# 3b/3bz

Hardware: AMD Instinct MI355X
Metric: decompressed MB/s on 1 GiB many-block zlib, 1/2/4/8 MI355X; % HBM roofline (higher is better)
Workload: dtype u8

## Files before the change

3bz_amd/csrc/tbz_engine.hpp:

```cpp
#pragma once
#include <algorithm>
#include <atomic>
#include <chrono>
#include <condition_variable>
#include <mutex>
#include <cstdio>
#include <cstdlib>
#include <cstring>
#include <functional>
#include <memory>
#include <string>
#include <thread>
#include <utility>
#include <vector>

#include "../../include/tbz_amd.h"
#include "tbz_kernels.hpp"

static_assert(sizeof(tbz_result) == 64, "tbz_result is exchanged between ranks as 64-octet records");
namespace tbz {

struct DevBuf {
  void* p = nullptr;
  size_t cap = 0;
};

}

#define TBZ_CTX_POOLS(X) \
  X(d_str_off) X(d_str_len) X(d_tile_first) X(d_tile_counts) X(d_tile_offsets) X(d_markers) X(d_items) X(d_res) \
  X(d_tok) X(d_scratch) X(d_runs) X(d_segs) X(d_groups) X(d_order) X(d_k3_fi) X(d_k3_ni) \
  X(d_k3_oo) X(d_k3_oc) X(d_k3_sums) X(d_k3_flags) X(d_k3_gscan) X(d_k3_gne) X(d_k3_streams) X(d_k3_glob) \
  X(d_redo_items) X(d_redo_res) X(d_k0_slots) X(d_k0_fm) X(d_hdr) X(d_gck) X(d_gchunks) X(d_ck_l1) \
  X(d_tok2) X(d_runs2) X(d_ck_chunks) X(d_ck_parts) X(d_ck_streams) X(d_ck_out) X(d_crc_tab) X(d_in_stage) \
  X(d_out_stage) X(d_kb_tf) X(d_kb_slots) X(d_kb_counts) X(d_kb_offsets) X(d_kb_cands) X(d_kb_fc) X(d_kb_head) \
  X(d_markers2) X(d_kb_fm2) X(d_mark) X(d_hg) X(d_k6s) X(d_bigs) X(d_recs) X(d_kc_tf) \
  X(d_kc_slots) X(d_kc_ends) X(d_kc_link) X(d_kc_fm2) X(d_markers3) X(d_kb_keep) X(d_kb_kcounts) X(d_gz_cands) \
  X(d_gz_count) X(d_gz_tmp) X(d_wide_res) X(d_cold) X(d_cold2) X(d_small_rec) \
  X(d_bit_off) X(d_ix_span) X(d_ix_recs) X(d_rec_pieces) X(d_rec_queries) X(d_rec_out) \
  X(d_srch_pieces) X(d_srch_flags) X(d_srch_hits)

namespace tbz {
static inline void cpu_relax() {
#if defined(__x86_64__) || defined(__i386__)
  __builtin_ia32_pause();
#else
  std::this_thread::yield();
// ... 72 lines not shown
      std::lock_guard<std::mutex> lk(mu);
      stop = true;
    }
    cv.notify_all();
    for (auto& t : th) t.join();
  }
};
}

struct tbz_ctx {
  int device = 0;
  hipStream_t stream = nullptr;
  hipStream_t stream2 = nullptr;
  hipEvent_t evw[2] = {};
  hipEvent_t ev[12] = {};
  std::string err;
  tbz_timings tim{};
  uint64_t gang_rounds = 0, gang_valid = 0;
  bool k1h = true;
  bool k2_ring2 = false;
  bool k2_single = false;
  bool host_layout = false;
  void* h_pin = nullptr;
  size_t h_pin_cap = 0;
  void* h_stage[4] = {};
  hipEvent_t ev_stage[4] = {};
  tbz::CopyPool* copy_pool = nullptr;
  tbz::CopyPool* copy_pool2 = nullptr;
  hipStream_t stream_in = nullptr, stream_out = nullptr;
  bool small_fused = true;
// ... 424 lines not shown
    R->trailer_isize = format == TBZ_FORMAT_GZIP ? q.trailer1 : 0u;
    (format == TBZ_FORMAT_ZLIB ? R->adler32 : R->crc32) = h->check;
  }
  ctx->tim.huff_launches = 1;
  ctx->tim.k1_gang = 64;
  ctx->tim.k2_kinds = q.tok_words ? 4u : 0u;
  ctx->tim.token_words = q.tok_words;
  ctx->tim.n_segments = ctx->tim.n_groups = R->segments;
  ctx->tim.scratch_bytes = scratch_total(ctx);
  ctx->gang_rounds = q.reserved >> 32;
  ctx->gang_valid = q.reserved & 0xffffffffu;
  *handled = true;
  return 0;
}

static void launch_k2_linear(tbz_ctx* ctx, K2Params& k2, size_t n_groups, uint64_t max_out) {
  k2.win_bytes = (u32)((max_out + K2_SLACK + 63) & ~63ull);
  ctx->tim.k2_kinds |= ctx->k2_single ? 2u : 1u;
  if (ctx->k2_single)
    TBZ_LAUNCH_DYN(tbz_k2_lz77_small, n_groups, k2.win_bytes + 2 * K2_TOKBUF + 512, ctx->stream, k2);
  else
    TBZ_LAUNCH_DYN_WG(tbz_k2_lz77_dual, n_groups, 128, k2.win_bytes + 2 * K2_TOKBUF + 512 + 2 * sizeof(K2Hand),
                      ctx->stream, k2);
}
static void launch_k2_ring(tbz_ctx* ctx, const K2Params& k2, size_t nwg) {
  ctx->tim.k2_kinds |= 4u;
  if (ctx->k2_single) TBZ_LAUNCH(tbz_k2_lz77, nwg, ctx->stream, k2);
  else if (ctx->k2_ring2) TBZ_LAUNCH_WG(tbz_k2_lz77_ring2, nwg, 128, ctx->stream, k2);
  else TBZ_LAUNCH_WG(tbz_k2_lz77_ring3, nwg, 192, ctx->stream, k2);
}
static void k2_trace(tbz_ctx* ctx) {
#ifdef TBZ_WAVE_TRACE
  if (const char* vp = getenv("TBZ_K2_TRACE")) {
    std::vector<u64> h(8192 * 8);
    hipStreamSynchronize(ctx->stream);
    u32 cn[4] = {0, 0, 0, 0};
    hipMemcpyFromSymbol(cn, HIP_SYMBOL(tbz_dbg_cnt), 16);
    fprintf(stderr, "tbz: K2 resolve since the start: %u batches with matches, %.2f rounds and %.1f matches per batch\n", cn[0],
            cn[0] ? (double)cn[1] / cn[0] : 0.0, cn[0] ? (double)cn[2] / cn[0] : 0.0);
    hipMemcpyFromSymbol(h.data(), HIP_SYMBOL(tbz_dbg), h.size() * 8);
    if (FILE* f = fopen(vp, "wb")) { fwrite(h.data(), 8, h.size(), f); fclose(f); }
  }
#endif
}
// ... 119 lines not shown
    if (total / count >= (uint64_t)ctx->tun.k6_lds_min) {
      q.pieces = (u32)((maxlen + 15 + K6R_PIECE - 1) / K6R_PIECE);
      TBZ_LAUNCH_WG(tbz_k6_resolve_lds, count * (size_t)q.pieces, K6R_THREADS, ctx->stream, q);
    } else {
      q.pieces = (u32)((maxlen + 15 + K6_PIECE - 1) / K6_PIECE);
      TBZ_LAUNCH(tbz_k6_resolve, count * (size_t)q.pieces, ctx->stream, q);
    }
  };
  resolve(o3s, r3s, K6_W);
  resolve(o3a, r3a, K6_W);
  resolve(o3b, r3b, 65536);
  TBZ_HIP(hipEventRecord(ctx->ev[11], ctx->stream));
  return 0;
}

enum { DIST_NONE = 0, DIST_FIRST = 1, DIST_AFTER_OVERFLOW = 2 };
struct Call {
  tbz_ctx* ctx;
  int format;
  size_t n;
  const void* d_in;
  const uint64_t *in_offs, *in_lens;
  void* d_out;
  const uint64_t *out_offs, *out_caps;
  tbz_result* results;
  bool size_only;
  CoreOpts* opt;
  std::vector<uint64_t> hist;
  std::vector<uint32_t> bit_off;
  const u32* d_bit_off = nullptr;
// ... 5 lines not shown
  std::vector<StreamPlan> sp;
  uint64_t tiles = 0, in_lo = ~0ull, in_extent = 0, in_total_bits = 0;
  uint32_t n_mark = 0, n_fixed_items = 0;
  uint32_t n_stored_heads = 0;
  std::vector<uint32_t> first_marker;
  const u64* d_markers_cur = nullptr;
  const u32* d_first_marker = nullptr;
  size_t n_items = 0;
  std::vector<Item> items;
  bool have_find = false;
  uint64_t pool_base = 0, pool2_base = 0, pool2_hi = 0;
  u32 half1 = 0, half2 = 0;
  bool wide_beside = false;
  float huff_ms = 0;
  bool simple = false;
  K3Params k3{};
  K3Global* h_glob = nullptr;
  K3Stream* h_k3s = nullptr;
  bool fused_adler = false;
  std::vector<std::vector<SegHost>> per_stream;
  std::vector<uint8_t> dist_first;
  uint64_t dist_at = ~0ull;
  std::vector<Seg> h_segs;
  std::vector<Group> h_groups;
  std::vector<uint8_t> h_hist;
  std::vector<uint32_t> h_gstream;
  std::vector<int32_t> h_grec;
  std::vector<BigSeg> bigs;
  uint32_t n_recs = 0;
};
// ... 66 lines not shown
    S.in_len = c.in_lens[s];
    S.out_off = c.size_only ? 0 : c.out_offs[s];
    S.out_cap = c.size_only ? ~0ull : c.out_caps[s];
    c.in_extent = std::max(c.in_extent, c.in_offs[s] + c.in_lens[s]);
    if (c.in_lens[s]) c.in_lo = std::min(c.in_lo, c.in_offs[s]);
    c.in_total_bits += c.in_lens[s] * 8;
    tile_first[s] = (uint32_t)c.tiles;
    c.tiles += ((((uintptr_t)c.d_in + c.in_offs[s]) & 15) + c.in_lens[s] + SCAN_TILE - 1) / SCAN_TILE;
    if (c.tiles > 0x7fffffffu) return TBZ_E_ARG;
  }
  tile_first[n] = (uint32_t)c.tiles;
  if (c.in_extent && !c.d_in) return TBZ_E_ARG;
  const size_t tiles = c.tiles;
  int r;
  if ((r = record(ctx, 0))) return r;
  if ((r = pinned(ctx, (n + 5) * 4 + 16 + sizeof(K3Global) + (n + 1) * sizeof(K3Stream)))) return r;
  if (tiles) {
    const std::vector<uint64_t> h_off(c.in_offs, c.in_offs + n), h_len(c.in_lens, c.in_lens + n);
    if ((r = upload(ctx, ctx->d_str_off, h_off))) return r;
    if ((r = upload(ctx, ctx->d_str_len, h_len))) return r;
    if ((r = upload(ctx, ctx->d_tile_first, tile_first))) return r;
    if ((r = ensure(ctx, ctx->d_tile_counts, tiles * 4))) return r;
    if ((r = ensure(ctx, ctx->d_tile_offsets, (tiles + 1) * 4))) return r;
    if ((r = ensure(ctx, ctx->d_k0_slots, tiles * (size_t)K0_SLOTS * 8))) return r;
    if ((r = ensure(ctx, ctx->d_markers, tiles * (size_t)K0_SLOTS * 8 + 16))) return r;
    if ((r = ensure(ctx, ctx->d_k0_fm, (n + 1) * 4 + 16))) return r;
    if ((r = ensure(ctx, ctx->d_items, (tiles * (size_t)K0_SLOTS + n) * sizeof(Item)))) return r;
    if (!c.bit_off.empty()) {
      if ((r = upload(ctx, ctx->d_bit_off, c.bit_off))) return r;
      c.d_bit_off = (const u32*)ctx->d_bit_off.p;
    }
// ... 241 lines not shown
  }
  return 0;
}
static u32 items_per_wg(size_t n_it) {
  u32 ipw = 64;
  while (ipw > 1 && n_it / ipw < 512) ipw >>= 1;
  return ipw;
}
static u32 pool_half(const Call& c, bool fix) { return fix ? c.half2 : c.half1; }
static u16* pool_tok(const Call& c, bool fix) {
  return fix ? (u16*)c.ctx->d_tok2.p - ((c.pool2_base >> c.half2) & ~7ull) : (u16*)c.ctx->d_tok.p - ((c.pool_base >> c.half1) & ~7ull);
}
static RunRec* pool_runs(const Call& c, bool fix) {
  return fix ? (RunRec*)c.ctx->d_runs2.p - (c.pool2_base >> RUN_SHIFT) : (RunRec*)c.ctx->d_runs.p - (c.pool_base >> RUN_SHIFT);
}
static int launch_lane(Call& c, const Item* d_items, SegResult* d_res, size_t n_it, bool fix, bool explicit_items = false) {
  tbz_ctx* ctx = c.ctx;
  if (pool_half(c, fix) && !explicit_items) return TBZ_E_INTERNAL;
  int rr = ensure(ctx, ctx->d_scratch, n_it * (size_t)K1_SCRATCH);
  if (rr) return rr;
  K1Params k1{(const u8*)c.d_in, pool_tok(c, fix), d_items, d_res, c.d_markers_cur,
              (u8*)ctx->d_scratch.p, pool_runs(c, fix), c.d_first_marker, (u32)c.n_mark, (u32)n_it, items_per_wg(n_it), c.resume_abs};
  TBZ_LAUNCH(tbz_k1_huff_decode, (n_it + k1.items_per_wg - 1) / k1.items_per_wg, ctx->stream, k1);
  return 0;
}
static u32 sub_min(const tbz_ctx* ctx) {
  if (ctx->tun.sub_min) return (u32)std::max(64, ctx->tun.sub_min & ~63);
  return KG_SUB_MIN;
}
static u64 wide_for(const tbz_ctx* ctx, int G, bool fix) {
  if (ctx->tun.wide_bits >= 0) return (u64)ctx->tun.wide_bits;
  if (ctx->k1_mode || fix || G >= 64) return 0;
  return (u64)G * KG_SUB_MAX * 2;
}
static u32 ovl_for(const tbz_ctx* ctx, int G) {
  if (ctx->tun.ovl) return (u32)std::max(64, ctx->tun.ovl);
  return G >= 32 ? 1024u : 768u;
}
// ... 38 lines not shown
    if (sub.empty()) continue;
    if (ctx->tun.debug && how == REDO_GANG) {
      uint64_t mx = 0;
      for (const Item& q : sub) mx = std::max<uint64_t>(mx, std::min(q.limit_bit, q.end_byte * 8) - q.start_bit);
      fprintf(stderr, "tbz: %zu large item(s) handed to gangs of 64 (the largest: %llu bits)\n", sub.size(), (unsigned long long)mx);
    }
    if (ctx->tun.debug && how == REDO_GANG_OWN) fprintf(stderr, "tbz: %zu item(s) decoded again into regions of their own\n", sub.size());
    if (ctx->tun.debug && how == REDO_LANE) fprintf(stderr, "tbz: %zu item(s) redone by the one-lane kernel\n", sub.size());
    std::vector<SegResult> tmp;
    int r;
    if ((r = k1_again(c, sub, how, fix, tmp))) return r;
    for (size_t k = 0; k < idx.size(); k++) rs[idx[k]] = tmp[k];
  }
  return 0;
}
static int launch_k1(Call& c, const Item* d_items, SegResult* d_res, size_t n_it, bool fix) {
  tbz_ctx* ctx = c.ctx;
  int G = k1_gang(c, n_it);
  if (G == 1 && pool_half(c, fix)) G = 8;
  if (!fix) ctx->tim.k1_gang = (uint32_t)G;
  if (G == 1) return launch_lane(c, d_items, d_res, n_it, fix);
  size_t per = 64 / G, nwg = (n_it + per - 1) / per;
  if (!fix && G <= 16 && wide_for(ctx, G, fix) && ctx->stream2) {
    int rr = ensure(ctx, ctx->d_wide_res, n_it * sizeof(SegResult));
    if (rr) return rr;
    if ((rr = ensure(ctx, ctx->d_cold2, n_it * (size_t)KG_COLD_STRIDE))) return rr;
    TBZ_HIP(hipEventRecord(ctx->evw[0], ctx->stream));
    TBZ_HIP(hipStreamWaitEvent(ctx->stream2, ctx->evw[0], 0));
    K1gParams kw = k1g_params(c, d_items, (SegResult*)ctx->d_wide_res.p, n_it, 64, fix, false, (u8*)ctx->d_cold2.p);
    kw.only_wide = 1;
    kw.wide_bits = wide_for(ctx, G, fix);
    TBZ_LAUNCH(tbz_k1g64_huff_decode, n_it, ctx->stream2, kw);
    TBZ_HIP(hipEventRecord(ctx->evw[1], ctx->stream2));
    c.wide_beside = true;
  }
  int rr;
  if ((rr = ensure(ctx, ctx->d_scratch, n_it * (size_t)K1_SCRATCH))) return rr;
  if ((rr = ensure(ctx, ctx->d_hdr, n_it * sizeof(HdrRec)))) return rr;
  if (G >= 32 && (rr = ensure(ctx, ctx->d_cold, n_it * (size_t)KG_COLD_STRIDE))) return rr;
  K1hParams kh{(const u8*)c.d_in, d_items, (u8*)ctx->d_scratch.p, (HdrRec*)ctx->d_hdr.p, (u32)n_it};
  if (ctx->k1h) TBZ_LAUNCH(tbz_k1h_headers, (n_it + 63) / 64, ctx->stream, kh);
  K1gParams kg = k1g_params(c, d_items, d_res, n_it, G, fix, false, (u8*)ctx->d_cold.p);
  kg.hdr = ctx->k1h ? (const HdrRec*)ctx->d_hdr.p : nullptr;
  kg.hdr_lens = (const u8*)ctx->d_scratch.p;
  kg.wide_bits = wide_for(ctx, G, fix);
#ifdef TBZ_WAVE_TRACE
  {
    static int n_launch = 0;
    u32 ef = (n_launch++ >= 1 && getenv("TBZ_EXP")) ? (u32)atoi(getenv("TBZ_EXP")) : 0u;
    hipMemcpyToSymbolAsync(HIP_SYMBOL(tbz_exp_flags), &ef, 4, 0, hipMemcpyHostToDevice, ctx->stream);
    hipStreamSynchronize(ctx->stream);
  }
  static u64* d_trace = nullptr;
  static size_t trace_wg = 0;
  if (const char* tp = getenv("TBZ_WAVE_TRACE")) {
    if (d_trace && trace_wg) {
      std::vector<u64> h(trace_wg * 16);
      hipStreamSynchronize(ctx->stream);
      hipMemcpy(h.data(), d_trace, h.size() * 8, hipMemcpyDeviceToHost);
      if (FILE* f = fopen(tp, "wb")) { fwrite(h.data(), 8, h.size(), f); fclose(f); }
      hipFree(d_trace);
    }
    hipMalloc((void**)&d_trace, nwg * 128);
    hipMemsetAsync(d_trace, 0, nwg * 128, ctx->stream);
    trace_wg = nwg;
    kg.trace = d_trace;
  }
#endif
  switch (G) {
    case 8: TBZ_LAUNCH(tbz_k1g8_huff_decode, nwg, ctx->stream, kg); break;
    case 16: TBZ_LAUNCH(tbz_k1g16_huff_decode, nwg, ctx->stream, kg); break;
    case 32: TBZ_LAUNCH(tbz_k1g32_huff_decode, nwg, ctx->stream, kg); break;
    default: TBZ_LAUNCH(tbz_k1g64_huff_decode, nwg, ctx->stream, kg); break;
  }
  if (c.wide_beside && !fix) TBZ_HIP(hipStreamWaitEvent(ctx->stream, ctx->evw[1], 0));
  return 0;
}

static int call_k1(Call& c) {
  tbz_ctx* ctx = c.ctx;
  const size_t n = c.n, n_items = c.n_items;
  const bool try_simple = !c.host_layout && n_items != 0;
  const u32 k3_tiles = (u32)((n_items + K3_TILE - 1) / K3_TILE);
  int r;
  if (try_simple) {
    std::vector<uint32_t> fi(n), ni(n);
    std::vector<uint64_t> oo(n), oc(n);
    for (size_t s = 0; s < n; s++) {
      fi[s] = c.sp[s].first_item;
      ni[s] = c.sp[s].n_items;
      oo[s] = c.sp[s].out_off;
      oc[s] = c.size_only ? 0 : c.sp[s].out_cap;
    }
    if ((r = upload(ctx, ctx->d_k3_fi, fi))) return r;
    if ((r = upload(ctx, ctx->d_k3_ni, ni))) return r;
    if ((r = upload(ctx, ctx->d_k3_oo, oo))) return r;
    if ((r = upload(ctx, ctx->d_k3_oc, oc))) return r;
    if ((r = ensure(ctx, ctx->d_k3_sums, 3 * (size_t)(k3_tiles + 1) * 8))) return r;
    if ((r = ensure(ctx, ctx->d_k3_flags, 4 * (size_t)k3_tiles * 8))) return r;
    if ((r = ensure(ctx, ctx->d_k3_gscan, n_items * 8))) return r;
    if ((r = ensure(ctx, ctx->d_k3_gne, n_items * 4))) return r;
    if ((r = ensure(ctx, ctx->d_segs, n_items * sizeof(Seg)))) return r;
    if ((r = ensure(ctx, ctx->d_groups, n_items * sizeof(Group)))) return r;
    if ((r = ensure(ctx, ctx->d_k3_streams, (n + 1) * sizeof(K3Stream)))) return r;
    if ((r = ensure(ctx, ctx->d_k3_glob, sizeof(K3Global)))) return r;
    c.k3 = K3Params{(const Item*)ctx->d_items.p, (const SegResult*)ctx->d_res.p, (const u32*)ctx->d_k3_fi.p,
                    (const u32*)ctx->d_k3_ni.p, (const u64*)ctx->d_k3_oo.p, (const u64*)ctx->d_k3_oc.p,
                    (u64*)ctx->d_k3_sums.p, (u64*)ctx->d_k3_flags.p, (u64*)ctx->d_k3_gscan.p, (u32*)ctx->d_k3_gne.p,
                    (Seg*)ctx->d_segs.p, (Group*)ctx->d_groups.p, (K3Stream*)ctx->d_k3_streams.p,
                    (K3Global*)ctx->d_k3_glob.p, (u32)n_items, k3_tiles, (u32)n};
  }
  if ((r = record(ctx, 2))) return r;
  if ((r = launch_k1(c, (const Item*)ctx->d_items.p, (SegResult*)ctx->d_res.p, n_items, false))) return r;
  TBZ_HIP(hipGetLastError());
  if ((r = record(ctx, 3))) return r;
  ctx->tim.huff_launches = 1;
  char* pin_k3 = (char*)ctx->h_pin + (((n + 5) * 4 + 15) & ~(size_t)15);
  c.h_glob = (K3Global*)pin_k3;
  c.h_k3s = (K3Stream*)(pin_k3 + sizeof(K3Global));
  if (!try_simple) return 0;
  TBZ_LAUNCH(tbz_k3_tile_sums, k3_tiles, ctx->stream, c.k3);
  TBZ_LAUNCH(tbz_k3_scan_tiles, 1, ctx->stream, c.k3);
  if ((r = read_back(ctx, c.h_glob, ctx->d_k3_glob.p, sizeof(K3Global)))) return r;
  c.simple = c.h_glob->not_simple == 0;
  if (c.simple && ctx->sym_hist && !c.size_only) {
    uint64_t target = std::max<uint64_t>(64u << 10, c.h_glob->total_out / 4096);
    if (ctx->tun.slice) target = std::max(1024, ctx->tun.slice);
    if (c.h_glob->max_out >= 2 * target) c.simple = false;
  }
  return 0;
}
static int32_t fill_result(Call& c, size_t s, int32_t status, uint32_t nseg, bool error_first = false) {
  StreamPlan& S = c.sp[s];
  tbz_result& R = c.results[s];
// ... 26 lines not shown
  }
  S.hdr_bit = (uint64_t)q.trailer0 | ((uint64_t)q.trailer1 << 32);
  if (q.pad == 1 && !(q.end_bit & 7)) {
    S.boundary_bit = q.end_bit;
    S.boundary_out = S.total_out;
  }
}
static int alloc_out(Call& c, const uint64_t& total, hipEvent_t ready = nullptr) {
  tbz_ctx* ctx = c.ctx;
  if (c.size_only || !c.opt || !c.opt->alloc) return 0;
  if (ready) TBZ_HIP(hipEventSynchronize(ready));
  c.d_out = c.opt->alloc(total);
  return c.d_out ? 0 : TBZ_E_NOMEM;
}

static int call_device_layout(Call& c) {
  tbz_ctx* ctx = c.ctx;
  const size_t n = c.n;
  const K3Global* g = c.h_glob;
  int r;
  TBZ_LAUNCH(tbz_k3_scan_items, c.k3.n_tiles, ctx->stream, c.k3);
  TBZ_LAUNCH(tbz_k3_emit, c.k3.n_tiles, ctx->stream, c.k3);
  TBZ_HIP(hipMemcpyAsync(c.h_k3s, ctx->d_k3_streams.p, (n + 1) * sizeof(K3Stream), hipMemcpyDeviceToHost, ctx->stream));
  TBZ_HIP(hipEventRecord(ctx->ev[7], ctx->stream));
  if ((r = record(ctx, 4))) return r;
  if ((r = alloc_out(c, c.h_k3s[0].total_out, ctx->ev[7]))) return r;
  if (!c.size_only) {
    if (!c.d_out) return TBZ_E_ARG;
    const u32 n_it = (u32)c.n_items;
    c.fused_adler = c.format == TBZ_FORMAT_ZLIB && !ctx->k2_single && g->n_big == 0 && !ctx->tun.no_fused_adler;
// ... 6 lines not shown
        if ((r = ensure(ctx, ctx->d_gchunks, (size_t)n_it * sizeof(CkChunk)))) return r;
        k2.gck = (CkPartial*)ctx->d_gck.p;
        k2.gchunks = (CkChunk*)ctx->d_gchunks.p;
      }
      launch_k2_linear(ctx, k2, n_it, g->max_small);
    }
    k2_trace(ctx);
    if (g->n_big) {
      k2.win_bytes = 0;
      k2.cls = g->n_big < n_it ? 2 : 0;
      launch_k2_ring(ctx, k2, n_it);
    }
    TBZ_HIP(hipGetLastError());
  }
  if ((r = record(ctx, 5))) return r;
  TBZ_HIP(hipEventSynchronize(ctx->ev[7]));
  c.huff_ms = elapsed(ctx, 2, 3);
  ctx->tim.huff_ms = c.huff_ms;
  ctx->tim.token_words = c.h_k3s[n].tok_words;
  ctx->tim.n_segments = ctx->tim.n_groups = c.h_k3s[n].nonempty;
  for (size_t s = 0; s < n; s++) {
    StreamPlan& S = c.sp[s];
    const K3Stream& k = c.h_k3s[s];
    S.total_out = k.total_out;
    S.saw_final = k.last.status == SEG_FINAL;
    S.trailer0 = k.last.trailer0;
    S.trailer1 = k.last.trailer1;
    S.trailer_have = k.last.trailer_have;
    S.in_end_bit = k.last.end_bit;
    S.boundary_bit = (S.n_items > 1 && !(k.last_start & 7)) ? k.last_start : 0;
    S.boundary_out = k.total_out - k.last.out_bytes;
    if (k.last.status == SEG_UNDERRUN) note_underrun(S, k.last, k.last_start);
    S.status = S.saw_final ? TBZ_FINISHED : TBZ_INPUT_UNDERRUN;
    S.done = true;
    fill_result(c, s, S.status, (uint32_t)k.nonempty);
  }
  return 0;
}

static int call_host_results(Call& c, std::vector<SegResult>& res) {
  tbz_ctx* ctx = c.ctx;
  const size_t n_items = c.n_items;
  int r;
  if (c.items.empty()) {
    c.items.resize(n_items);
    if ((r = read_back(ctx, c.items.data(), ctx->d_items.p, n_items * sizeof(Item)))) return r;
  }
  res.resize(n_items);
  if ((r = read_back(ctx, res.data(), ctx->d_res.p, res.size() * sizeof(SegResult)))) return r;
  c.huff_ms = elapsed(ctx, 2, 3);
  if (c.wide_beside && std::any_of(res.begin(), res.end(), [](const SegResult& q) { return q.status == SEG_WIDE; })) {
    std::vector<SegResult> wr(n_items);
// ... 439 lines not shown
  return 0;
}

static int inflate_core(tbz_ctx* ctx, int format, size_t n, const void* d_in, const uint64_t* in_offs,
                        const uint64_t* in_lens, void* d_out, const uint64_t* out_offs, const uint64_t* out_caps,
                        tbz_result* results, bool size_only, CoreOpts* opt = nullptr) {
  Call c{ctx, format, n, d_in, in_offs, in_lens, d_out, out_offs, out_caps, results, size_only, opt};
  bool done = false;
  int r;
  if ((r = call_begin(c, &done)) || done) return r;
  if ((r = call_k0(c))) return r;
  if ((r = call_k0b(c))) return r;
  if ((r = call_k0c(c))) return r;
  if ((r = call_pools(c))) return r;
  if ((r = call_k1(c))) return r;
  if (c.simple) {
    if ((r = call_device_layout(c))) return r;
  } else {
    std::vector<SegResult> res;
    if ((r = call_host_results(c, res))) return r;
    if ((r = call_chain_walk(c, res))) return r;
    if ((r = call_distance(c))) return r;
    if ((r = call_groups(c))) return r;
    if ((r = call_host_k2(c))) return r;
  }
  return call_finish(c);
}

}

extern "C" {
// ... 93 lines not shown
    t.debug2 = getenv("TBZ_DEBUG2") != nullptr;
    if (const char* m = getenv("TBZ_DEBUG_CANDS")) t.debug_cands = m;
  }
  if (const char* m = getenv("TBZ_COPY_THREADS")) ctx->copy_threads = std::max(1, std::min(64, atoi(m)));
  if (const char* m = getenv("TBZ_STAGE_CHUNK_KIB")) ctx->stage_chunk = (size_t)std::max(64, atoi(m)) << 10;
  if (const char* m = getenv("TBZ_SMALL_FUSED")) ctx->small_fused = m[0] != '0';
  if (const char* m = getenv("TBZ_SMALL_MAX_KIB")) ctx->small_max_in = (size_t)std::max(0, atoi(m)) << 10;
  if (const char* m = getenv("TBZ_PIPE_MIN_KIB")) ctx->pipe_min = (size_t)std::max(0, atoi(m)) << 10;
  if (const char* m = getenv("TBZ_PIPE_PART_KIB")) ctx->pipe_part = (size_t)std::max(16, atoi(m)) << 10;
  ctx->copy_threads = std::min<int>(ctx->copy_threads, std::max(1u, std::thread::hardware_concurrency()));
  if (const char* m = getenv("TBZ_HOST_LAYOUT")) ctx->host_layout = m[0] == '1';
  if (const char* m = getenv("TBZ_K2_MODE")) ctx->k2_single = !strcmp(m, "single");
  if (const char* m = getenv("TBZ_K2_RING")) ctx->k2_ring2 = !strcmp(m, "2");
  if (const char* m = getenv("TBZ_K1H")) ctx->k1h = m[0] != '0';
  if (const char* m = getenv("TBZ_HIST")) ctx->sym_hist = strcmp(m, "off") != 0;
  if (const char* m = getenv("TBZ_POOL_CAP_MIB")) ctx->pool_cap = (uint64_t)std::max(1, atoi(m)) << 20;
  if (const char* m = getenv("TBZ_FIND")) ctx->find_mode = !strcmp(m, "off") ? 0 : !strcmp(m, "always") ? 2 : 1;
  ctx->k1_mode = k1_mode;
  *out_ctx = ctx;
  return 0;
}

void tbz_ctx_destroy(tbz_ctx* ctx) {
  if (!ctx) return;
  hipSetDevice(ctx->device);
  if (ctx->stream) hipStreamSynchronize(ctx->stream);
  for (auto* b : tbz::all_pools(ctx))
    if (b->p) hipFree(b->p);
  for (auto& b : ctx->dense)
    if (b.p) hipFree(b.p);
  if (ctx->h_pin) hipHostFree(ctx->h_pin);
  delete ctx->copy_pool;
  delete ctx->copy_pool2;
  if (ctx->stream_in) hipStreamDestroy(ctx->stream_in);
  if (ctx->stream_out) hipStreamDestroy(ctx->stream_out);
  for (int k = 0; k < 4; k++) {
    if (ctx->h_stage[k]) hipHostFree(ctx->h_stage[k]);
    if (ctx->ev_stage[k]) hipEventDestroy(ctx->ev_stage[k]);
  }
  for (auto& ev : ctx->ev)
    if (ev) hipEventDestroy(ev);
  for (auto& ev : ctx->evw)
    if (ev) hipEventDestroy(ev);
  if (ctx->stream2) hipStreamDestroy(ctx->stream2);
  if (ctx->stream) hipStreamDestroy(ctx->stream);
  delete ctx;
}

const char* tbz_last_error(const tbz_ctx* ctx) { return ctx ? ctx->err.c_str() : "no context"; }

int tbz_last_timings(const tbz_ctx* ctx, tbz_timings* out) {
  if (!ctx || !out) return TBZ_E_ARG;
  *out = ctx->tim;
  return 0;
}

static int inflate_passes(tbz_ctx* ctx, int format, size_t n, const void* d_in, const uint64_t* in_offs,
// ... 2434 lines not shown
```

3bz_amd/csrc/tbz_kernels.hpp:

```cpp
#pragma once
#include "tbz_platform.hpp"
#include "tbz_structs.hpp"

namespace tbz {

constexpr i32 E_BTYPE = -1, E_STORED_LEN = -2, E_OVERSUB = -3, E_INCOMPLETE = -4, E_REPEAT_NO_PREV = -5,
              E_REPEAT_OVERRUN = -6, E_INVALID_CODE = -7, E_ZLIB_HEADER = -9, E_ZLIB_DICT = -10,
              E_GZIP_MAGIC = -12, E_GZIP_METHOD = -13, E_GZIP_FLAGS = -14, E_GZIP_HCRC = -15, E_TREE_OVERFLOW = -18;

TBZ_DEV u32 wave_incl_scan_u32(u32 v) { return tbz_wave_incl_scan_u32(v); }
TBZ_DEV u64 wave_incl_scan_u64(u64 v) {
  const u32 lane = tbz_lane();
#pragma unroll
  for (u32 d = 1; d < 64; d <<= 1) {
    u64 t = tbz_shfl_up64(v, d);
    if (lane >= d) v += t;
  }
  return v;
}
TBZ_DEV u64 wave_sum_u64(u64 v) {
#pragma unroll
  for (int m = 32; m >= 1; m >>= 1) v += tbz_shfl_xor64(v, m);
  return v;
}
// ... 3073 lines not shown
  const u32* order;
  const u8* in_base;
  u8* out_base;
  u32 n_groups;
  u32 win_bytes;
  u32 cls;
  CkPartial* gck;
  CkChunk* gchunks;
  u32 hist;
  u32 plane;
  u64 out_bias;
  u32 mixed;
  u32 n_plain;
  u8* mark_base;
  u64 mark_bias;
};

template <class W>
TBZ_DEV u32 ring(u32 x) { return W::LINEAR ? x : (x >= W::RW ? x - W::RW : x); }

template <class W>
TBZ_DEV void k2_flush(const u8* win, u8* outp, u64 from, u64 to, u64 clip, u32 a0) {
  constexpr bool LINEAR = W::LINEAR;
  constexpr u32 RW = LINEAR ? 1u : W::RW;
  if (to > clip) to = clip;
  if (from >= to) return;
  const u32 lane = tbz_lane();
  tbz_sync();
  u64 head_end = ((from + a0 + 15) & ~15ull) - a0;
  if (head_end > to) head_end = to;
// ... 263 lines not shown
  const bool fastable = len <= K2_SHORT && dist >= len && (LINEAR || (rs + 32 <= RW && rd + 32 <= RW));
  const i64 s = (i64)gpos + dofs - (i64)dist;
  tbz_sync();
  u64 oddq = 0;
  if (!W::LINEAR) {
    u64 oddm;
    pend &= ~k2_far_round<W, STAGE != K2_NEAR>(S, pend, rpos, gpos, dofs, len, dist, mine, rd, s, oddm);
    if (STAGE == K2_FAR) return;
    oddq = oddm & pend;
  }
  k2_rounds<W>(S, pend, oddq, rpos, gpos, dofs, len, dist, rd, rs, need, fastable, longm);
}


TBZ_DEV bool k2_pick_group(const K2Params& P, u32& gi, Group& g, Seg& sg_guess, u32 at = ~0u) {
  if (at == ~0u) at = tbz_block();
  if (at >= P.n_groups) return false;
  gi = P.order ? P.order[at] : at;
  sg_guess = P.segs[gi];
  g = P.groups[gi];
  if (!P.order && P.cls) {
    const bool small = (g.seg_first == gi ? sg_guess : P.segs[g.seg_first]).out_bytes + K2_SLACK <= K2_SMALL_MAX;
    if ((P.cls == 1) != small) return false;
  }
  return true;
}

template <class W, u32 SPAN, u32 DUAL, class Emit, class Finish>
TBZ_DEV void k2_body(const K2Params& P, u32 gi, const Group& g, const Seg& sg_guess, u8* win, u16* tks,
                     u32* rcache, Emit&& emit, Finish&& finish) {
  constexpr bool LINEAR = W::LINEAR;
// ... 787 lines not shown
  const Item* items;
  const SegResult* res;
  const u32* first_item;
  const u32* n_items_s;
  const u64* out_off;
  const u64* out_cap;
  u64* tile_sums;
  u64* tile_flags;
  u64* gscan;
  u32* gne;
  Seg* segs;
  Group* groups;
  K3Stream* streams;
  K3Global* glob;
  u32 n_items, n_tiles, n_streams;
};

TBZ_KERNEL void tbz_k3_tile_sums(K3Params P) {
  const u32 lane = tbz_lane(), t = tbz_block();
  u64 so = 0, sw = 0, sn = 0, bad = 0, nbig = 0, mx = 0, mxo = 0;
  for (u32 it = 0; it < K3_TILE / 64; it++) {
    const u32 i = t * K3_TILE + it * 64 + lane;
    if (i >= P.n_items) continue;
    const SegResult q = P.res[i];
    const u32 s = P.items[i].stream;
    const bool last = i - P.first_item[s] == P.n_items_s[s] - 1;
    const bool ok = (q.status == (last ? SEG_FINAL : SEG_LANDED) || (last && q.status == SEG_UNDERRUN)) && q.max_deficit == 0;
    bad |= ok ? 0u : 1u;
    so += q.out_bytes;
    sw += q.tok_words;
    sn += (q.out_bytes | q.tok_words) ? 1u : 0u;
    const bool big = q.out_bytes + K2_SLACK > K2_SMALL_MAX;
    nbig += big ? 1u : 0u;
    mx = !big && q.out_bytes > mx ? q.out_bytes : mx;
// ... 14 lines not shown
  if (lane == 0) {
    const u32 T1 = P.n_tiles + 1;
    P.tile_sums[t] = so;
    P.tile_sums[T1 + t] = sw;
    P.tile_sums[2 * T1 + t] = sn;
    P.tile_flags[t] = bad;
    P.tile_flags[P.n_tiles + t] = nbig;
    P.tile_flags[2 * P.n_tiles + t] = mx;
    P.tile_flags[3 * P.n_tiles + t] = mxo;
  }
}

TBZ_KERNEL void tbz_k3_scan_tiles(K3Params P) {
  const u32 lane = tbz_lane();
  const u32 T1 = P.n_tiles + 1;
  for (u32 c = 0; c < 3; c++) {
    u64 carry = 0;
    for (u32 i = 0; i < P.n_tiles; i += 64) {
      const u64 v = (i + lane) < P.n_tiles ? P.tile_sums[c * T1 + i + lane] : 0;
      const u64 inc = wave_incl_scan_u64(v);
      if ((i + lane) < P.n_tiles) P.tile_sums[c * T1 + i + lane] = carry + inc - v;
      carry += tbz_shfl64(inc, 63);
    }
    if (lane == 0) P.tile_sums[c * T1 + P.n_tiles] = carry;
  }
  u64 bad = 0, nbig = 0, mx = 0, mxo = 0;
  for (u32 i = lane; i < P.n_tiles; i += 64) {
    bad += P.tile_flags[i];
    nbig += P.tile_flags[P.n_tiles + i];
    const u64 m = P.tile_flags[2 * P.n_tiles + i];
    mx = m > mx ? m : mx;
    const u64 m2 = P.tile_flags[3 * P.n_tiles + i];
    mxo = m2 > mxo ? m2 : mxo;
  }
  bad = wave_sum_u64(bad);
  nbig = wave_sum_u64(nbig);
#pragma unroll
  for (int m = 32; m >= 1; m >>= 1) {
    const u64 o = tbz_shfl_xor64(mx, m);
    mx = o > mx ? o : mx;
    const u64 o2 = tbz_shfl_xor64(mxo, m);
    mxo = o2 > mxo ? o2 : mxo;
  }
  if (lane == 0) {
    K3Global gl;
    gl.not_simple = bad ? 1u : 0u;
    gl.n_big = (u32)nbig;
    gl.max_small = mx;
    gl.max_out = mxo;
    gl.total_out = P.tile_sums[P.n_tiles];
    *P.glob = gl;
  }
}

TBZ_KERNEL void tbz_k3_scan_items(K3Params P) {
  const u32 lane = tbz_lane(), t = tbz_block();
  u64 carry = P.tile_sums[t];
  u32 carry_ne = (u32)P.tile_sums[2 * (P.n_tiles + 1) + t];
  for (u32 it = 0; it < K3_TILE / 64; it++) {
    const u32 i = t * K3_TILE + it * 64 + lane;
    u64 v = 0;
    u32 ne = 0;
    if (i < P.n_items) {
      const SegResult q = P.res[i];
      v = q.out_bytes;
      ne = (q.out_bytes | q.tok_words) ? 1u : 0u;
    }
    const u64 inc = wave_incl_scan_u64(v);
    const u32 inc_ne = wave_incl_scan_u32(ne);
    if (i < P.n_items) {
      P.gscan[i] = carry + inc - v;
      P.gne[i] = carry_ne + inc_ne - ne;
    }
    carry += tbz_shfl64(inc, 63);
    carry_ne += tbz_shfl(inc_ne, 63);
  }
}

TBZ_KERNEL void tbz_k3_emit(K3Params P) {
  const u32 lane = tbz_lane(), t = tbz_block();
  const u32 T1 = P.n_tiles + 1;
  for (u32 it = 0; it < K3_TILE / 64; it++) {
    const u32 i = t * K3_TILE + it * 64 + lane;
    if (i >= P.n_items) continue;
    const SegResult q = P.res[i];
    const Item im = P.items[i];
    const u32 s = im.stream, f = P.first_item[s];
    const u64 rel = P.gscan[i] - P.gscan[f];
    Seg sg;
    sg.tok = q.tok;
    sg.tok_words = q.tok_words;
    sg.out_bytes = q.out_bytes;
    sg.n_runs = q.n_runs;
    sg.run_first = 0;
    sg.runs = q.runs;
// ... 3 lines not shown
    g.out_abs = P.out_off[s] + rel;
    g.out_end = P.out_off[s] + P.out_cap[s];
    g.seg_first = i;
    g.seg_count = 1;
    P.groups[i] = g;
    if (i - f == P.n_items_s[s] - 1) {
      K3Stream st;
      st.total_out = rel + q.out_bytes;
      st.tok_words = 0;
      st.nonempty = P.gne[i] - P.gne[f] + ((q.out_bytes | q.tok_words) ? 1u : 0u);
      st.last = q;
      st.last_start = im.start_bit;
      P.streams[s] = st;
    }
  }
  if (t == 0 && lane == 0) {
    K3Stream tot;
    tot.total_out = P.tile_sums[P.n_tiles];
    tot.tok_words = P.tile_sums[T1 + P.n_tiles];
    tot.nonempty = P.tile_sums[2 * T1 + P.n_tiles];
    tot.last = SegResult{};
    tot.last_start = 0;
    P.streams[P.n_streams] = tot;
  }
}

struct BigSeg {
  Seg seg;
  u64 out_abs;
  u64 out_end;
  u64 target;
// ... 917 lines not shown
```

Before: 206,100.

## Pipeline Huffman decode and LZ77 resolve across tile partitions on two streams

Splits the item range into partitions by K3 tiles and runs Huffman decode (K1), the tile scans and emit (K3), and LZ77 resolve (K2) for each partition on alternating streams. Later partitions' decode can then overlap earlier partitions' LZ77 work. Tile scans carry their prefix sums between partitions through a small device buffer, and events serialize the scan and emit steps in partition order. The cost is one host sync per partition for its verdict, more launches, and a fallback path when a partition turns out not to be simple.

Result: faster. 209,800, median of 6 (+1.8%).

```diff
diff --git a/3bz_amd/csrc/tbz_engine.hpp b/3bz_amd/csrc/tbz_engine.hpp
--- a/3bz_amd/csrc/tbz_engine.hpp
+++ b/3bz_amd/csrc/tbz_engine.hpp
@@ -30,7 +30,7 @@
 #define TBZ_CTX_POOLS(X) \
   X(d_str_off) X(d_str_len) X(d_tile_first) X(d_tile_counts) X(d_tile_offsets) X(d_markers) X(d_items) X(d_res) \
   X(d_tok) X(d_scratch) X(d_runs) X(d_segs) X(d_groups) X(d_order) X(d_k3_fi) X(d_k3_ni) \
-  X(d_k3_oo) X(d_k3_oc) X(d_k3_sums) X(d_k3_flags) X(d_k3_gscan) X(d_k3_gne) X(d_k3_streams) X(d_k3_glob) \
+  X(d_k3_oo) X(d_k3_oc) X(d_k3_sums) X(d_k3_flags) X(d_k3_gscan) X(d_k3_gne) X(d_k3_streams) X(d_k3_glob) X(d_k3_carry) \
   X(d_redo_items) X(d_redo_res) X(d_k0_slots) X(d_k0_fm) X(d_hdr) X(d_gck) X(d_gchunks) X(d_ck_l1) \
   X(d_tok2) X(d_runs2) X(d_ck_chunks) X(d_ck_parts) X(d_ck_streams) X(d_ck_out) X(d_crc_tab) X(d_in_stage) \
   X(d_out_stage) X(d_kb_tf) X(d_kb_slots) X(d_kb_counts) X(d_kb_offsets) X(d_kb_cands) X(d_kb_fc) X(d_kb_head) \
@@ -133,6 +133,9 @@
   hipStream_t stream2 = nullptr;
   hipEvent_t evw[2] = {};
   hipEvent_t ev[12] = {};
+  std::vector<hipEvent_t> ev_k12;
+  int k12_parts = 2;
+  size_t k12_min_items = 32768;
   std::string err;
   tbz_timings tim{};
   uint64_t gang_rounds = 0, gang_valid = 0;
@@ -587,20 +590,21 @@
   return 0;
 }
 
-static void launch_k2_linear(tbz_ctx* ctx, K2Params& k2, size_t n_groups, uint64_t max_out) {
+static void launch_k2_linear(tbz_ctx* ctx, K2Params& k2, size_t n_groups, uint64_t max_out, hipStream_t st = nullptr) {
+  if (!st) st = ctx->stream;
   k2.win_bytes = (u32)((max_out + K2_SLACK + 63) & ~63ull);
   ctx->tim.k2_kinds |= ctx->k2_single ? 2u : 1u;
   if (ctx->k2_single)
-    TBZ_LAUNCH_DYN(tbz_k2_lz77_small, n_groups, k2.win_bytes + 2 * K2_TOKBUF + 512, ctx->stream, k2);
+    TBZ_LAUNCH_DYN(tbz_k2_lz77_small, n_groups, k2.win_bytes + 2 * K2_TOKBUF + 512, st, k2);
   else
-    TBZ_LAUNCH_DYN_WG(tbz_k2_lz77_dual, n_groups, 128, k2.win_bytes + 2 * K2_TOKBUF + 512 + 2 * sizeof(K2Hand),
-                      ctx->stream, k2);
-}
-static void launch_k2_ring(tbz_ctx* ctx, const K2Params& k2, size_t nwg) {
+    TBZ_LAUNCH_DYN_WG(tbz_k2_lz77_dual, n_groups, 128, k2.win_bytes + 2 * K2_TOKBUF + 512 + 2 * sizeof(K2Hand), st, k2);
+}
+static void launch_k2_ring(tbz_ctx* ctx, const K2Params& k2, size_t nwg, hipStream_t st = nullptr) {
+  if (!st) st = ctx->stream;
   ctx->tim.k2_kinds |= 4u;
-  if (ctx->k2_single) TBZ_LAUNCH(tbz_k2_lz77, nwg, ctx->stream, k2);
-  else if (ctx->k2_ring2) TBZ_LAUNCH_WG(tbz_k2_lz77_ring2, nwg, 128, ctx->stream, k2);
-  else TBZ_LAUNCH_WG(tbz_k2_lz77_ring3, nwg, 192, ctx->stream, k2);
+  if (ctx->k2_single) TBZ_LAUNCH(tbz_k2_lz77, nwg, st, k2);
+  else if (ctx->k2_ring2) TBZ_LAUNCH_WG(tbz_k2_lz77_ring2, nwg, 128, st, k2);
+  else TBZ_LAUNCH_WG(tbz_k2_lz77_ring3, nwg, 192, st, k2);
 }
 static void k2_trace(tbz_ctx* ctx) {
 #ifdef TBZ_WAVE_TRACE
@@ -750,6 +754,7 @@
   return 0;
 }
 
+constexpr u32 K12_MAX_PARTS = 64;
 enum { DIST_NONE = 0, DIST_FIRST = 1, DIST_AFTER_OVERFLOW = 2 };
 struct Call {
   tbz_ctx* ctx;
@@ -785,6 +790,7 @@
   bool wide_beside = false;
   float huff_ms = 0;
   bool simple = false;
+  bool k12 = false;
   K3Params k3{};
   K3Global* h_glob = nullptr;
   K3Stream* h_k3s = nullptr;
@@ -881,7 +887,7 @@
   const size_t tiles = c.tiles;
   int r;
   if ((r = record(ctx, 0))) return r;
-  if ((r = pinned(ctx, (n + 5) * 4 + 16 + sizeof(K3Global) + (n + 1) * sizeof(K3Stream)))) return r;
+  if ((r = pinned(ctx, (n + 5) * 4 + 16 + (1 + K12_MAX_PARTS) * sizeof(K3Global) + (n + 1) * sizeof(K3Stream)))) return r;
   if (tiles) {
     const std::vector<uint64_t> h_off(c.in_offs, c.in_offs + n), h_len(c.in_lens, c.in_lens + n);
     if ((r = upload(ctx, ctx->d_str_off, h_off))) return r;
@@ -1153,14 +1159,21 @@
 static RunRec* pool_runs(const Call& c, bool fix) {
   return fix ? (RunRec*)c.ctx->d_runs2.p - (c.pool2_base >> RUN_SHIFT) : (RunRec*)c.ctx->d_runs.p - (c.pool_base >> RUN_SHIFT);
 }
-static int launch_lane(Call& c, const Item* d_items, SegResult* d_res, size_t n_it, bool fix, bool explicit_items = false) {
+struct K1Part {
+  size_t slot0, n_slots;
+  hipStream_t stream;
+  int gang;
+};
+static int launch_lane(Call& c, const Item* d_items, SegResult* d_res, size_t n_it, bool fix, bool explicit_items = false,
+                       const K1Part* part = nullptr) {
   tbz_ctx* ctx = c.ctx;
   if (pool_half(c, fix) && !explicit_items) return TBZ_E_INTERNAL;
-  int rr = ensure(ctx, ctx->d_scratch, n_it * (size_t)K1_SCRATCH);
+  int rr = ensure(ctx, ctx->d_scratch, (part ? part->n_slots : n_it) * (size_t)K1_SCRATCH);
   if (rr) return rr;
   K1Params k1{(const u8*)c.d_in, pool_tok(c, fix), d_items, d_res, c.d_markers_cur,
-              (u8*)ctx->d_scratch.p, pool_runs(c, fix), c.d_first_marker, (u32)c.n_mark, (u32)n_it, items_per_wg(n_it), c.resume_abs};
-  TBZ_LAUNCH(tbz_k1_huff_decode, (n_it + k1.items_per_wg - 1) / k1.items_per_wg, ctx->stream, k1);
+              (u8*)ctx->d_scratch.p + (part ? part->slot0 : 0) * (size_t)K1_SCRATCH, pool_runs(c, fix), c.d_first_marker,
+              (u32)c.n_mark, (u32)n_it, items_per_wg(n_it), c.resume_abs};
+  TBZ_LAUNCH(tbz_k1_huff_decode, (n_it + k1.items_per_wg - 1) / k1.items_per_wg, part ? part->stream : ctx->stream, k1);
   return 0;
 }
 static u32 sub_min(const tbz_ctx* ctx) {
@@ -1229,14 +1242,23 @@
   }
   return 0;
 }
-static int launch_k1(Call& c, const Item* d_items, SegResult* d_res, size_t n_it, bool fix) {
-  tbz_ctx* ctx = c.ctx;
+static int k1_gang_of(const Call& c, size_t n_it, bool fix) {
   int G = k1_gang(c, n_it);
   if (G == 1 && pool_half(c, fix)) G = 8;
+  return G;
+}
+static bool k1_wide_beside(const Call& c, int G, bool fix) {
+  return !fix && G > 1 && G <= 16 && wide_for(c.ctx, G, fix) && c.ctx->stream2;
+}
+static int launch_k1(Call& c, const Item* d_items, SegResult* d_res, size_t n_it, bool fix, const K1Part* part = nullptr) {
+  tbz_ctx* ctx = c.ctx;
+  const int G = part ? part->gang : k1_gang_of(c, n_it, fix);
+  [[maybe_unused]] const hipStream_t st = part ? part->stream : ctx->stream;
+  const size_t slot0 = part ? part->slot0 : 0, n_slots = part ? part->n_slots : n_it;
   if (!fix) ctx->tim.k1_gang = (uint32_t)G;
-  if (G == 1) return launch_lane(c, d_items, d_res, n_it, fix);
+  if (G == 1) return launch_lane(c, d_items, d_res, n_it, fix, false, part);
   size_t per = 64 / G, nwg = (n_it + per - 1) / per;
-  if (!fix && G <= 16 && wide_for(ctx, G, fix) && ctx->stream2) {
+  if (!part && k1_wide_beside(c, G, fix)) {
     int rr = ensure(ctx, ctx->d_wide_res, n_it * sizeof(SegResult));
     if (rr) return rr;
     if ((rr = ensure(ctx, ctx->d_cold2, n_it * (size_t)KG_COLD_STRIDE))) return rr;
@@ -1250,14 +1272,17 @@
     c.wide_beside = true;
   }
   int rr;
-  if ((rr = ensure(ctx, ctx->d_scratch, n_it * (size_t)K1_SCRATCH))) return rr;
-  if ((rr = ensure(ctx, ctx->d_hdr, n_it * sizeof(HdrRec)))) return rr;
-  if (G >= 32 && (rr = ensure(ctx, ctx->d_cold, n_it * (size_t)KG_COLD_STRIDE))) return rr;
-  K1hParams kh{(const u8*)c.d_in, d_items, (u8*)ctx->d_scratch.p, (HdrRec*)ctx->d_hdr.p, (u32)n_it};
-  if (ctx->k1h) TBZ_LAUNCH(tbz_k1h_headers, (n_it + 63) / 64, ctx->stream, kh);
-  K1gParams kg = k1g_params(c, d_items, d_res, n_it, G, fix, false, (u8*)ctx->d_cold.p);
-  kg.hdr = ctx->k1h ? (const HdrRec*)ctx->d_hdr.p : nullptr;
-  kg.hdr_lens = (const u8*)ctx->d_scratch.p;
+  if ((rr = ensure(ctx, ctx->d_scratch, n_slots * (size_t)K1_SCRATCH))) return rr;
+  if ((rr = ensure(ctx, ctx->d_hdr, n_slots * sizeof(HdrRec)))) return rr;
+  if (G >= 32 && (rr = ensure(ctx, ctx->d_cold, n_slots * (size_t)KG_COLD_STRIDE))) return rr;
+  u8* const scratch = (u8*)ctx->d_scratch.p + slot0 * (size_t)K1_SCRATCH;
+  HdrRec* const hdr = (HdrRec*)ctx->d_hdr.p + slot0;
+  u8* const cold = ctx->d_cold.p ? (u8*)ctx->d_cold.p + slot0 * (size_t)KG_COLD_STRIDE : nullptr;
+  K1hParams kh{(const u8*)c.d_in, d_items, scratch, hdr, (u32)n_it};
+  if (ctx->k1h) TBZ_LAUNCH(tbz_k1h_headers, (n_it + 63) / 64, st, kh);
+  K1gParams kg = k1g_params(c, d_items, d_res, n_it, G, fix, false, cold);
+  kg.hdr = ctx->k1h ? hdr : nullptr;
+  kg.hdr_lens = scratch;
   kg.wide_bits = wide_for(ctx, G, fix);
 #ifdef TBZ_WAVE_TRACE
   {
@@ -1283,15 +1308,17 @@
   }
 #endif
   switch (G) {
-    case 8: TBZ_LAUNCH(tbz_k1g8_huff_decode, nwg, ctx->stream, kg); break;
-    case 16: TBZ_LAUNCH(tbz_k1g16_huff_decode, nwg, ctx->stream, kg); break;
-    case 32: TBZ_LAUNCH(tbz_k1g32_huff_decode, nwg, ctx->stream, kg); break;
-    default: TBZ_LAUNCH(tbz_k1g64_huff_decode, nwg, ctx->stream, kg); break;
+    case 8: TBZ_LAUNCH(tbz_k1g8_huff_decode, nwg, st, kg); break;
+    case 16: TBZ_LAUNCH(tbz_k1g16_huff_decode, nwg, st, kg); break;
+    case 32: TBZ_LAUNCH(tbz_k1g32_huff_decode, nwg, st, kg); break;
+    default: TBZ_LAUNCH(tbz_k1g64_huff_decode, nwg, st, kg); break;
   }
   if (c.wide_beside && !fix) TBZ_HIP(hipStreamWaitEvent(ctx->stream, ctx->evw[1], 0));
   return 0;
 }
 
+static u32 k12_parts(const Call& c, u32 k3_tiles);
+static int call_k12(Call& c, u32 parts);
 static int call_k1(Call& c) {
   tbz_ctx* ctx = c.ctx;
   const size_t n = c.n, n_items = c.n_items;
@@ -1318,21 +1345,26 @@
     if ((r = ensure(ctx, ctx->d_segs, n_items * sizeof(Seg)))) return r;
     if ((r = ensure(ctx, ctx->d_groups, n_items * sizeof(Group)))) return r;
     if ((r = ensure(ctx, ctx->d_k3_streams, (n + 1) * sizeof(K3Stream)))) return r;
-    if ((r = ensure(ctx, ctx->d_k3_glob, sizeof(K3Global)))) return r;
+    if ((r = ensure(ctx, ctx->d_k3_glob, (1 + K12_MAX_PARTS) * sizeof(K3Global)))) return r;
+    if ((r = ensure(ctx, ctx->d_k3_carry, 3 * 8))) return r;
     c.k3 = K3Params{(const Item*)ctx->d_items.p, (const SegResult*)ctx->d_res.p, (const u32*)ctx->d_k3_fi.p,
                     (const u32*)ctx->d_k3_ni.p, (const u64*)ctx->d_k3_oo.p, (const u64*)ctx->d_k3_oc.p,
                     (u64*)ctx->d_k3_sums.p, (u64*)ctx->d_k3_flags.p, (u64*)ctx->d_k3_gscan.p, (u32*)ctx->d_k3_gne.p,
                     (Seg*)ctx->d_segs.p, (Group*)ctx->d_groups.p, (K3Stream*)ctx->d_k3_streams.p,
-                    (K3Global*)ctx->d_k3_glob.p, (u32)n_items, k3_tiles, (u32)n};
+                    (K3Global*)ctx->d_k3_glob.p, (u32)n_items, k3_tiles, (u32)n, 0, k3_tiles, (u64*)ctx->d_k3_carry.p};
   }
   if ((r = record(ctx, 2))) return r;
+  char* pin_k3 = (char*)ctx->h_pin + (((n + 5) * 4 + 15) & ~(size_t)15);
+  c.h_glob = (K3Global*)pin_k3;
+  c.h_k3s = (K3Stream*)(pin_k3 + sizeof(K3Global));
+  if (try_simple) {
+    const u32 parts = k12_parts(c, k3_tiles);
+    if (parts > 1) return call_k12(c, parts);
+  }
   if ((r = launch_k1(c, (const Item*)ctx->d_items.p, (SegResult*)ctx->d_res.p, n_items, false))) return r;
   TBZ_HIP(hipGetLastError());
   if ((r = record(ctx, 3))) return r;
   ctx->tim.huff_launches = 1;
-  char* pin_k3 = (char*)ctx->h_pin + (((n + 5) * 4 + 15) & ~(size_t)15);
-  c.h_glob = (K3Global*)pin_k3;
-  c.h_k3s = (K3Stream*)(pin_k3 + sizeof(K3Global));
   if (!try_simple) return 0;
   TBZ_LAUNCH(tbz_k3_tile_sums, k3_tiles, ctx->stream, c.k3);
   TBZ_LAUNCH(tbz_k3_scan_tiles, 1, ctx->stream, c.k3);
@@ -1389,6 +1421,7 @@
   return c.d_out ? 0 : TBZ_E_NOMEM;
 }
 
+static int device_layout_results(Call& c);
 static int call_device_layout(Call& c) {
   tbz_ctx* ctx = c.ctx;
   const size_t n = c.n;
@@ -1425,6 +1458,11 @@
     TBZ_HIP(hipGetLastError());
   }
   if ((r = record(ctx, 5))) return r;
+  return device_layout_results(c);
+}
+static int device_layout_results(Call& c) {
+  tbz_ctx* ctx = c.ctx;
+  const size_t n = c.n;
   TBZ_HIP(hipEventSynchronize(ctx->ev[7]));
   c.huff_ms = elapsed(ctx, 2, 3);
   ctx->tim.huff_ms = c.huff_ms;
@@ -1447,6 +1485,120 @@
     fill_result(c, s, S.status, (uint32_t)k.nonempty);
   }
   return 0;
+}
+
+static u32 k12_parts(const Call& c, u32 k3_tiles) {
+  const tbz_ctx* ctx = c.ctx;
+  if (ctx->k12_parts <= 1 || c.size_only || (c.opt && c.opt->alloc) || !c.d_out || c.n_items < ctx->k12_min_items) return 1;
+  if (k1_wide_beside(c, k1_gang_of(c, c.n_items, false), false)) return 1;
+  const u32 want = std::min<u32>((u32)ctx->k12_parts, K12_MAX_PARTS), per = (k3_tiles + want - 1) / want;
+  return (k3_tiles + per - 1) / per;
+}
+static int call_k12(Call& c, u32 parts) {
+  tbz_ctx* ctx = c.ctx;
+  const size_t n = c.n, n_items = c.n_items;
+  const u32 tiles = c.k3.n_tiles, per = (tiles + parts - 1) / parts;
+  const int G = k1_gang_of(c, n_items, false);
+  const bool zlib_partials = c.format == TBZ_FORMAT_ZLIB && !ctx->k2_single && !ctx->tun.no_fused_adler;
+  int r;
+  while (ctx->ev_k12.size() < 3 * (size_t)parts) {
+    hipEvent_t e;
+    TBZ_HIP(hipEventCreate(&e));
+    ctx->ev_k12.push_back(e);
+  }
+  hipEvent_t* const ev_tiles = ctx->ev_k12.data();
+  hipEvent_t* const ev_verdict = ev_tiles + parts;
+  hipEvent_t* const ev_emit = ev_verdict + parts;
+  if (zlib_partials) {
+    if ((r = ensure(ctx, ctx->d_gck, n_items * sizeof(CkPartial)))) return r;
+    if ((r = ensure(ctx, ctx->d_gchunks, n_items * sizeof(CkChunk)))) return r;
+  }
+  const hipStream_t S[2] = {ctx->stream, ctx->stream2};
+  TBZ_HIP(hipEventRecord(ctx->evw[0], ctx->stream));
+  TBZ_HIP(hipStreamWaitEvent(ctx->stream2, ctx->evw[0], 0));
+  K3Global* const h_parts = (K3Global*)(c.h_k3s + (n + 1));
+  K3Global* const d_parts = (K3Global*)ctx->d_k3_glob.p + 1;
+  auto k3_of = [&](u32 p) {
+    K3Params k = c.k3;
+    k.t0 = p * per;
+    k.t1 = std::min(tiles, k.t0 + per);
+    k.glob = d_parts + p;
+    return k;
+  };
+  auto enqueue = [&](u32 p, bool with_k3) -> int {
+    const hipStream_t st = S[p & 1];
+    const K3Params k = k3_of(p);
+    const size_t i0 = (size_t)k.t0 * K3_TILE, i1 = std::min(n_items, (size_t)k.t1 * K3_TILE);
+    const K1Part kp{i0, n_items, st, G};
+    int rr = launch_k1(c, (const Item*)ctx->d_items.p + i0, (SegResult*)ctx->d_res.p + i0, i1 - i0, false, &kp);
+    if (rr) return rr;
+    if (p == parts - 1) {
+      TBZ_HIP(hipEventRecord(ctx->ev[3], st));
+      TBZ_HIP(hipEventRecord(ctx->ev[4], st));
+    }
+    if (!with_k3) return 0;
+    TBZ_LAUNCH(tbz_k3_tile_sums, k.t1 - k.t0, st, k);
+    if (p) TBZ_HIP(hipStreamWaitEvent(st, ev_tiles[p - 1], 0));
+    TBZ_LAUNCH(tbz_k3_scan_tiles, 1, st, k);
+    TBZ_HIP(hipEventRecord(ev_tiles[p], st));
+    TBZ_HIP(hipMemcpyAsync(h_parts + p, d_parts + p, sizeof(K3Global), hipMemcpyDeviceToHost, st));
+    TBZ_HIP(hipEventRecord(ev_verdict[p], st));
+    return 0;
+  };
+  const uint64_t slice_floor = !ctx->sym_hist ? ~0ull : ctx->tun.slice ? 2 * (uint64_t)std::max(1024, ctx->tun.slice) : 128u << 10;
+  bool ok = true, partials = zlib_partials;
+  ctx->tim.huff_launches = parts;
+  if ((r = enqueue(0, true))) return r;
+  for (u32 p = 0; p < parts && ok; p++) {
+    const hipStream_t st = S[p & 1];
+    if (p + 1 < parts && (r = enqueue(p + 1, true))) return r;
+    TBZ_HIP(hipEventSynchronize(ev_verdict[p]));
+    const K3Global g = h_parts[p];
+    if (g.not_simple || g.max_out >= slice_floor) {
+      ok = false;
+      for (u32 q = p + 2; q < parts; q++)
+        if ((r = enqueue(q, false))) return r;
+      break;
+    }
+    const K3Params k = k3_of(p);
+    const u32 i0 = k.t0 * K3_TILE, i1 = (u32)std::min(n_items, (size_t)k.t1 * K3_TILE), n_it = i1 - i0;
+    if (p) TBZ_HIP(hipStreamWaitEvent(st, ev_emit[p - 1], 0));
+    TBZ_LAUNCH(tbz_k3_scan_items, k.t1 - k.t0, st, k);
+    TBZ_LAUNCH(tbz_k3_emit, k.t1 - k.t0, st, k);
+    TBZ_HIP(hipEventRecord(ev_emit[p], st));
+    if (p == parts - 1) {
+      TBZ_HIP(hipMemcpyAsync(c.h_k3s, ctx->d_k3_streams.p, (n + 1) * sizeof(K3Stream), hipMemcpyDeviceToHost, st));
+      TBZ_HIP(hipEventRecord(ctx->ev[7], st));
+    }
+    partials = partials && g.n_big == 0;
+    K2Params k2{(const Seg*)ctx->d_segs.p, (const Group*)ctx->d_groups.p, nullptr,
+                (const u8*)c.d_in, (u8*)c.d_out, i1, 0, 0, nullptr, nullptr, 0, 0, 0, 0, 0, nullptr, 0, i0};
+    if (g.n_big < n_it) {
+      k2.cls = g.n_big ? 1 : 0;
+      if (partials) {
+        k2.gck = (CkPartial*)ctx->d_gck.p;
+        k2.gchunks = (CkChunk*)ctx->d_gchunks.p;
+      }
+      launch_k2_linear(ctx, k2, n_it, g.max_small, st);
+    }
+    if (g.n_big) {
+      k2.win_bytes = 0;
+      k2.cls = g.n_big < n_it ? 2 : 0;
+      launch_k2_ring(ctx, k2, n_it, st);
+    }
+  }
+  TBZ_HIP(hipGetLastError());
+  TBZ_HIP(hipEventRecord(ctx->evw[1], ctx->stream2));
+  TBZ_HIP(hipStreamWaitEvent(ctx->stream, ctx->evw[1], 0));
+  if (!ok) {
+    c.simple = false;
+    ctx->tim.k2_kinds = 0;
+    return 0;
+  }
+  if ((r = record(ctx, 5))) return r;
+  c.simple = c.k12 = true;
+  c.fused_adler = partials;
+  return device_layout_results(c);
 }
 
 static int call_host_results(Call& c, std::vector<SegResult>& res) {
@@ -1916,7 +2068,8 @@
   if ((r = call_k0c(c))) return r;
   if ((r = call_pools(c))) return r;
   if ((r = call_k1(c))) return r;
-  if (c.simple) {
+  if (c.k12) {
+  } else if (c.simple) {
     if ((r = call_device_layout(c))) return r;
   } else {
     std::vector<SegResult> res;
@@ -2040,6 +2193,8 @@
   if (const char* m = getenv("TBZ_K2_RING")) ctx->k2_ring2 = !strcmp(m, "2");
   if (const char* m = getenv("TBZ_K1H")) ctx->k1h = m[0] != '0';
   if (const char* m = getenv("TBZ_HIST")) ctx->sym_hist = strcmp(m, "off") != 0;
+  if (const char* m = getenv("TBZ_K12_PARTS")) ctx->k12_parts = std::max(0, atoi(m));
+  if (const char* m = getenv("TBZ_K12_MIN_ITEMS")) ctx->k12_min_items = (size_t)std::max(1L, atol(m));
   if (const char* m = getenv("TBZ_POOL_CAP_MIB")) ctx->pool_cap = (uint64_t)std::max(1, atoi(m)) << 20;
   if (const char* m = getenv("TBZ_FIND")) ctx->find_mode = !strcmp(m, "off") ? 0 : !strcmp(m, "always") ? 2 : 1;
   ctx->k1_mode = k1_mode;
@@ -2067,6 +2222,8 @@
   for (auto& ev : ctx->ev)
     if (ev) hipEventDestroy(ev);
   for (auto& ev : ctx->evw)
+    if (ev) hipEventDestroy(ev);
+  for (auto& ev : ctx->ev_k12)
     if (ev) hipEventDestroy(ev);
   if (ctx->stream2) hipStreamDestroy(ctx->stream2);
   if (ctx->stream) hipStreamDestroy(ctx->stream);
diff --git a/3bz_amd/csrc/tbz_kernels.hpp b/3bz_amd/csrc/tbz_kernels.hpp
--- a/3bz_amd/csrc/tbz_kernels.hpp
+++ b/3bz_amd/csrc/tbz_kernels.hpp
@@ -3111,6 +3111,7 @@
   u32 n_plain;
   u8* mark_base;
   u64 mark_bias;
+  u32 first;
 };
 
 template <class W>
@@ -3404,7 +3405,7 @@
 
 
 TBZ_DEV bool k2_pick_group(const K2Params& P, u32& gi, Group& g, Seg& sg_guess, u32 at = ~0u) {
-  if (at == ~0u) at = tbz_block();
+  if (at == ~0u) at = tbz_block() + P.first;
   if (at >= P.n_groups) return false;
   gi = P.order ? P.order[at] : at;
   sg_guess = P.segs[gi];
@@ -4222,10 +4223,12 @@
   K3Stream* streams;
   K3Global* glob;
   u32 n_items, n_tiles, n_streams;
+  u32 t0, t1;
+  u64* carry;
 };
 
 TBZ_KERNEL void tbz_k3_tile_sums(K3Params P) {
-  const u32 lane = tbz_lane(), t = tbz_block();
+  const u32 lane = tbz_lane(), t = P.t0 + tbz_block();
   u64 so = 0, sw = 0, sn = 0, bad = 0, nbig = 0, mx = 0, mxo = 0;
   for (u32 it = 0; it < K3_TILE / 64; it++) {
     const u32 i = t * K3_TILE + it * 64 + lane;
@@ -4270,18 +4273,23 @@
 TBZ_KERNEL void tbz_k3_scan_tiles(K3Params P) {
   const u32 lane = tbz_lane();
   const u32 T1 = P.n_tiles + 1;
+  u64 total_out = 0;
   for (u32 c = 0; c < 3; c++) {
-    u64 carry = 0;
-    for (u32 i = 0; i < P.n_tiles; i += 64) {
-      const u64 v = (i + lane) < P.n_tiles ? P.tile_sums[c * T1 + i + lane] : 0;
+    u64 carry = P.t0 ? P.carry[c] : 0;
+    for (u32 i = P.t0; i < P.t1; i += 64) {
+      const u64 v = (i + lane) < P.t1 ? P.tile_sums[c * T1 + i + lane] : 0;
       const u64 inc = wave_incl_scan_u64(v);
-      if ((i + lane) < P.n_tiles) P.tile_sums[c * T1 + i + lane] = carry + inc - v;
+      if ((i + lane) < P.t1) P.tile_sums[c * T1 + i + lane] = carry + inc - v;
       carry += tbz_shfl64(inc, 63);
     }
-    if (lane == 0) P.tile_sums[c * T1 + P.n_tiles] = carry;
+    if (lane == 0) {
+      P.carry[c] = carry;
+      if (P.t1 == P.n_tiles) P.tile_sums[c * T1 + P.n_tiles] = carry;
+    }
+    if (c == 0) total_out = carry;
   }
   u64 bad = 0, nbig = 0, mx = 0, mxo = 0;
-  for (u32 i = lane; i < P.n_tiles; i += 64) {
+  for (u32 i = P.t0 + lane; i < P.t1; i += 64) {
     bad += P.tile_flags[i];
     nbig += P.tile_flags[P.n_tiles + i];
     const u64 m = P.tile_flags[2 * P.n_tiles + i];
@@ -4304,13 +4312,13 @@
     gl.n_big = (u32)nbig;
     gl.max_small = mx;
     gl.max_out = mxo;
-    gl.total_out = P.tile_sums[P.n_tiles];
+    gl.total_out = total_out;
     *P.glob = gl;
   }
 }
 
 TBZ_KERNEL void tbz_k3_scan_items(K3Params P) {
-  const u32 lane = tbz_lane(), t = tbz_block();
+  const u32 lane = tbz_lane(), t = P.t0 + tbz_block();
   u64 carry = P.tile_sums[t];
   u32 carry_ne = (u32)P.tile_sums[2 * (P.n_tiles + 1) + t];
   for (u32 it = 0; it < K3_TILE / 64; it++) {
@@ -4334,7 +4342,7 @@
 }
 
 TBZ_KERNEL void tbz_k3_emit(K3Params P) {
-  const u32 lane = tbz_lane(), t = tbz_block();
+  const u32 lane = tbz_lane(), t = P.t0 + tbz_block();
   const u32 T1 = P.n_tiles + 1;
   for (u32 it = 0; it < K3_TILE / 64; it++) {
     const u32 i = t * K3_TILE + it * 64 + lane;
@@ -4368,7 +4376,7 @@
       P.streams[s] = st;
     }
   }
-  if (t == 0 && lane == 0) {
+  if (t == P.n_tiles - 1 && lane == 0) {
     K3Stream tot;
     tot.total_out = P.tile_sums[P.n_tiles];
     tot.tok_words = P.tile_sums[T1 + P.n_tiles];
```
